# urgent-challenge/urgent2026_challenge_track1

Hardware: AMD Instinct MI355X
Metric: utterances/sec (4 s @ 48 kHz) train step (higher is better)
Workload: dtype bf16

## Files before the change

include/urse.h:

```cpp
#ifndef URSE_H_
#define URSE_H_
#include <stdint.h>

#ifdef __cplusplus
extern "C" {
#endif

#define URSE_OK 0
#define URSE_ERR_INVALID_ARG (-1)
#define URSE_ERR_LAUNCH (-2)
#define URSE_ERR_UNSUPPORTED (-3)
#define URSE_ERR_RUNTIME (-4)

#define URSE_F32 0
#define URSE_BF16 1
#define URSE_F16 2
#define URSE_BF16_ACT_F16 3

#define URSE_WIN_RECT 0
#define URSE_WIN_HANN 1

int urse_version(void);
const char* urse_last_error(void);

#define URSE_KV_NT_BRES 0
#define URSE_KV_NT_RING 1
#define URSE_KV_NT_RING_WIDE 2
#define URSE_KV_NT_128 3
#define URSE_KV_NT_GROUPED_RING 4
#define URSE_KV_NT_GROUPED_128 5
#define URSE_KV_TN_RING 6
#define URSE_KV_TN_RING_T 7
#define URSE_KV_TN_DUAL 8
#define URSE_KV_TN_128 9
#define URSE_KV_TN_GROUPED 10
#define URSE_KV_LSTM_FWD_STREAM 11
#define URSE_KV_LSTM_FWD_WIDE 12
#define URSE_KV_LSTM_FWD_CLUSTER 13
#define URSE_KV_LSTM_FWD_CLUSTER2 14
#define URSE_KV_LSTM_BWD_STREAM16 15
#define URSE_KV_LSTM_BWD_STREAM32 16
#define URSE_KV_LSTM_BWD_CLUSTER 17
#define URSE_KV_LSTM_BWD_SPLIT 18
#define URSE_KV_STFT960 19
#define URSE_KV_STFT_GENERIC 20
#define URSE_KV_ISTFT_GENERIC 21
#define URSE_KV_ISTFT960 22
#define URSE_KV_LSTM_FWD_RW 23
#define URSE_KV_TN_ACT_F16 24
#define URSE_KV_LSTM_FWD_RWX 25
#define URSE_KV_LSTM_BWD_NSPLIT 26
#define URSE_KV_LSTM_FWD_CLUSTERX 27
#define URSE_KV_COUNT 32
int urse_launch_count(int variant);
int urse_launch_counts_reset(void);

int urse_stft_fwd(const float* wav, const int32_t* lens, float* spec, int B, int L, int n_fft, int hop,
                  int window, void* stream);
int urse_istft_fwd(const float* spec, float* wav, int B, int T, int n_fft, int hop, int L_out, int window,
                   void* stream);
int urse_istft_bwd(const float* grad_wav, float* grad_spec, int B, int T, int n_fft, int hop, int L_out,
                   int window, void* stream);

int urse_gemm_nt(const void* A, int64_t lda, const void* B, int64_t ldb, void* C, int64_t ldc, const float* bias,
                 const float* resid, int64_t ldr, int64_t M, int64_t N, int64_t K, int in_dtype, int out_dtype,
                 int act, void* stream);
int urse_gemm_nt_gnstats(const void* A, int64_t lda, const void* B, int64_t ldb, float* C, int64_t ldc, const float* bias,
                         const float* resid, int64_t ldr, int64_t M, int64_t N, int64_t K, int in_dtype, int act,
                         double* stats, int64_t rows_per_group, void* stream);
int urse_gemm_nt_gnbwd(const void* A, int64_t lda, const void* B, int64_t ldb, float* C, int64_t M, int64_t N, int64_t K, int in_dtype,
                       const float* x, const double* stats, const float* gamma, double* sums, float* dgamma, float* dbeta, float* part,
                       int slots, int64_t rows_per_group, float eps, void* stream);
int urse_gemm_nt_grouped(const void* descs, int groups, int max_blocks, int in_dtype, int out_dtype, int act,
                         void* stream);
int urse_gemm_nt_grouped_h(const void* descs, const int64_t* host_descs, int groups, int in_dtype, int out_dtype,
                           int act, void* stream);
int urse_gemm_tn(const void* A, int64_t lda, const void* B, int64_t ldb, float* C, int64_t ldc, float* colsum,
                 int64_t R, int64_t Mo, int64_t No, int64_t shift, int64_t inner, int64_t period,
                 int64_t invalid_step, int64_t perm_h, int dtype, int target_workgroups, void* stream);
int urse_gemm_tn_act_f16_supported(int64_t R, int64_t Mo, int64_t No, int64_t No2, int with_colsum, int64_t inner, int64_t period);
int urse_gemm_tn_dual(const void* A, int64_t lda, const void* B, int64_t ldb, float* C, int64_t ldc, float* colsum,
                      const void* B2, int64_t ldb2, float* C2, int64_t ldc2, int64_t R, int64_t Mo, int64_t No, int64_t No2,
                      int64_t shift, int64_t inner, int64_t period, int64_t invalid_step, int64_t perm_h, int dtype,
                      int target_workgroups, void* stream);
int urse_gemm_tn_grouped(const void* descs, int groups, int max_blocks, int dtype, void* stream);
// ... 196 lines not shown
```

urgent2026_challenge_track1_amd/csrc/gemm.hip:

```cpp
#include <stdlib.h>

#include <type_traits>
#include "urse_common.h"

namespace urse {

typedef __bf16 bf16x8_t __attribute__((ext_vector_type(8)));
typedef short short8_t __attribute__((ext_vector_type(8)));
typedef short short4_t __attribute__((ext_vector_type(4)));
typedef float f32x4_t __attribute__((ext_vector_type(4)));

struct GemmDesc {
  const char* A;
  const char* B;
  char* C;
  const float* bias;
  const float* resid;
  long lda, ldb, ldc;
  long M, N, K;
  long ldr;
};

constexpr int BM = 128, BN = 128;
constexpr int SLAB = 64;
// ... 1150 lines not shown
    ++it_;
#endif
  }
  }
  asm volatile("s_waitcnt vmcnt(0)" ::: "memory");

#pragma unroll
  for (int j = 0; j < NT; ++j) {
    const long v = n0 + (wn * NT + j) * 16 + (lane & 15);
    float* dst = nullptr;
    long ld = 0, col = 0;
    if (v < p.No) { dst = p.C; ld = p.ldc; col = v; }
    else if (v >= No8 && v < V) { dst = p.C2; ld = p.ldc2; col = v - No8; }
    else if (v == vones) { dst = p.colsum; ld = 1; col = 0; }
    if (dst == nullptr) continue;
#pragma unroll
    for (int i = 0; i < MT; ++i)
#pragma unroll
      for (int r = 0; r < 4; ++r) {
        const long row = m0 + wm * (MT * 16) + i * 16 + (lane >> 4) * 4 + r;
        atomicAdd(dst + tn_perm(row, p.perm_h) * ld + col, acc[i][j][r]);
      }
  }
}

static void launch_tn_dma(int ntw, int csm, dim3 grid, hipStream_t st, const TnArgs& p, int cvt = 0) {
  if (cvt == 1) { hipLaunchKernelGGL((gemm_tn_dma_kernel<7, 2, 1>), grid, dim3(512), 0, st, p); return; }
#define URSE_TN_L(N_, C_) hipLaunchKernelGGL((gemm_tn_dma_kernel<N_, C_>), grid, dim3(512), 0, st, p)
  if (ntw == 7) { if (csm == 0) URSE_TN_L(7, 0); else if (csm == 1) URSE_TN_L(7, 1); else URSE_TN_L(7, 2); }
  else { if (csm == 0) URSE_TN_L(8, 0); else if (csm == 1) URSE_TN_L(8, 1); else URSE_TN_L(8, 2); }
#undef URSE_TN_L
}

struct NtExtra {
  double* gstats;
  long rpg;
  const float* gnb_x;
  const double* gnb_stats;
  const float* gnb_gamma;
  double* gnb_sums;
  float* gnb_part;
  int gnb_slots;
  float gnb_eps;
};

template <typename TO, int NTW, int ACT, int BMX, int WNC, int GNB = 0, typename TI = bf16_t>
__device__ __forceinline__ void gemm_nt_dma_body(const GemmDesc& d, double* gstats = nullptr, long rpg = 0, const NtExtra* xt = nullptr) {
  constexpr int BNX = 16 * NTW * WNC, NWV = BMX / 64 * WNC, NTHR = NWV * 64;
  constexpr int BNR = WNC == 2 ? 256 : 16 * NTW * WNC;
  constexpr int NST = NWV == 8 ? URSE_NT_NST : 3, STAGE = (BMX + BNR) * 64, BOFF = BMX * 64;
  constexpr int AI = (BMX / 16 + NWV - 1) / NWV;
  constexpr int BI = (BNR / 16 + NWV - 1) / NWV;
  constexpr int DPW = AI + BI;
  static_assert(AI * NWV * 16 == BMX, "A image blocks divide evenly over the waves");
  __shared__ __attribute__((aligned(1024))) char lds[NST * STAGE + 1024];
  const int tn = (int)((d.N + BNX - 1) / BNX), tm = (int)((d.M + BMX - 1) / BMX);
  if ((int)blockIdx.x >= tm * tn) return;
  const int bid = xcd_remap(blockIdx.x, tm * tn);
  const int tile_m = bid / tn, tile_n = bid - tile_m * tn;
  const long m0 = (long)tile_m * BMX, n0 = (long)tile_n * BNX;
  const int tid = threadIdx.x, lane = tid & 63;
  const int w = __builtin_amdgcn_readfirstlane(tid >> 6), wm = w / WNC, wn = w % WNC;
  const int nk = (int)(d.K / 32);
  const char* zsrc = reinterpret_cast<const char*>(g_tn_zero_page) + lane * 16;
  const int srow = lane >> 2, schunk = (lane & 3) ^ ((lane >> 3) & 3);
  const int lc = lane & 15, lr = lane >> 4;
// ... 175 lines not shown
            uint2 pk;
            pk.x = pack2<TO>(v[0], v[1]);
            pk.y = pack2<TO>(v[2], v[3]);
            *reinterpret_cast<uint2*>(dst) = pk;
          } else {
            *reinterpret_cast<f32x4_t*>(dst) = v;
          }
        }
      }
    }
    __syncthreads();
    if constexpr (GNB) {
      constexpr int SLOTS = NTHR / CPR, XI = (RPP + SLOTS - 1) / SLOTS;
      const int slot = tid / CPR, chf = tid - slot * CPR;
      const long col = n0 + chf * EPC;
#pragma unroll
      for (int i = GXA; i < XI; ++i) {
        const int lr_ = slot + i * SLOTS;
        const long row = m0 + pass * RPP + lr_;
        const bool ok = slot < SLOTS && col < d.N && lr_ < RPP && row < d.M;
        gnb_xpre[i] = ok ? *reinterpret_cast<const float4*>(xt->gnb_x + row * d.ldc + col) : make_float4(0.f, 0.f, 0.f, 0.f);
      }
      if (slot < SLOTS && col < d.N) {
#pragma unroll
        for (int i = 0; i < XI; ++i) {
          const int lr_ = slot + i * SLOTS;
          const long row = m0 + pass * RPP + lr_;
          if (lr_ < RPP && row < d.M) {
            const float4 f = *reinterpret_cast<const float4*>(lds + lr_ * CP + chf * 16);
            __builtin_nontemporal_store(*reinterpret_cast<const f32x4_t*>(&f), reinterpret_cast<f32x4_t*>(C + row * d.ldc + col));
            const float4 xv = gnb_xpre[i];
            const bool first = row < gnb_bound;
            const float mean = first ? gnb_m[0] : gnb_m[1], rstd = first ? gnb_r[0] : gnb_r[1];
            const float dy[4] = {f.x, f.y, f.z, f.w}, xs[4] = {xv.x, xv.y, xv.z, xv.w};
            float a1 = 0.f, a2 = 0.f;
#pragma unroll
            for (int q = 0; q < 4; ++q) {
              const float xh = (xs[q] - mean) * rstd;
              gnb_dg[q] += dy[q] * xh;
              gnb_db[q] += dy[q];
              a1 += dy[q] * gnb_ga[q];
              a2 += dy[q] * gnb_ga[q] * xh;
            }
            if (first) { gsa += a1; gqa += a2; } else { gsb += a1; gqb += a2; }
          }
        }
      }
      continue;
    }
    int lrow = tid / CPR, ch = tid - lrow * CPR;
    constexpr int DROW = NTHR / CPR, DCH = NTHR - DROW * CPR;
    for (; lrow < RPP; lrow += DROW) {
      const long row = m0 + pass * RPP + lrow, col = n0 + ch * EPC;
      if (row < d.M && col < d.N) {
        const char* src = lds + lrow * CP + ch * 16;
        if (vec_ok && col + EPC <= d.N) {
          uint4 v = *reinterpret_cast<const uint4*>(src);
          if (OS == 4 && d.resid && ACT != 2) {
            const float4 rr = *reinterpret_cast<const float4*>(d.resid + row * d.ldr + col);
            float4 f = *reinterpret_cast<float4*>(&v);
            f.x += rr.x; f.y += rr.y; f.z += rr.z; f.w += rr.w;
            v = *reinterpret_cast<uint4*>(&f);
          }
          if (gst) {
            const float4 f = *reinterpret_cast<const float4*>(&v);
            const float sv = (f.x + f.y) + (f.z + f.w), qv = (f.x * f.x + f.y * f.y) + (f.z * f.z + f.w * f.w);
            if (row < gbound) { gsa += sv; gqa += qv; } else { gsb += sv; gqb += qv; }
          }
#ifdef NABL_NO_GST
          if (v.x == 0x12345678u)
#endif
          __builtin_nontemporal_store(*reinterpret_cast<const f32x4_t*>(&v), reinterpret_cast<f32x4_t*>(C + row * d.ldc + col));
          if constexpr (C2K) {
            if (C2) {
              float a0, a1, a2, a3, a4, a5, a6, a7;
              unpack2<f16_t>(v.x, a0, a1); unpack2<f16_t>(v.y, a2, a3); unpack2<f16_t>(v.z, a4, a5); unpack2<f16_t>(v.w, a6, a7);
              const uint4 o = make_uint4(pack2<bf16_t>(a0, a1), pack2<bf16_t>(a2, a3), pack2<bf16_t>(a4, a5), pack2<bf16_t>(a6, a7));
              __builtin_nontemporal_store(*reinterpret_cast<const f32x4_t*>(&o), reinterpret_cast<f32x4_t*>(C2 + row * d.ldr + col));
            }
          }
        } else {
          const TO* sv = reinterpret_cast<const TO*>(src);
          for (int e = 0; e < EPC && col + e < d.N; ++e) {
            float f = to_f32<TO>(sv[e]);
            if (OS == 4 && d.resid && ACT != 2) f += d.resid[row * d.ldr + col + e];
            if (gst) {
              if (row < gbound) { gsa += f; gqa += f * f; } else { gsb += f; gqb += f * f; }
            }
            C[row * d.ldc + col + e] = from_f32<TO>(f);
            if constexpr (C2K) {
              if (C2) C2[row * d.ldr + col + e] = f32_to_bf16(f);
            }
          }
        }
      }
      ch += DCH;
      if (ch >= CPR) { ch -= CPR; ++lrow; }
    }
  }
// ... 30 lines not shown
        const float vg[4] = {sg.x, sg.y, sg.z, sg.w}, vb[4] = {sb.x, sb.y, sb.z, sb.w};
        for (int q = 0; q < 4 && col + q < d.N; ++q) {
          atomicAdd(part + col + q, vg[q]);
          atomicAdd(part + d.N + col + q, vb[q]);
        }
      }
    }
    return;
  }
  if (gst) {
    __syncthreads();
    double* red = reinterpret_cast<double*>(lds);
    const double r0 = wave_sum_d((double)gsa), r1 = wave_sum_d((double)gqa), r2 = wave_sum_d((double)gsb), r3 = wave_sum_d((double)gqb);
    if (lane == 0) { red[w * 4] = r0; red[w * 4 + 1] = r1; red[w * 4 + 2] = r2; red[w * 4 + 3] = r3; }
    __syncthreads();
    if (tid < 4) {
      double t = 0.0;
      for (int i = 0; i < NWV; ++i) t += red[i * 4 + tid];
      const long g = gidx + (tid >> 1);
      if (tid < 2 || gbound < m0 + BMX) {
        if (g * rpg < d.M) atomicAdd(gstats + g * 2 + (tid & 1), t);
      }
    }
  }
}

template <typename TO, int NTW, int ACT, int BMX, int WNC = 2, typename TI = bf16_t>
__global__ void __launch_bounds__(BMX / 64 * WNC * 64) gemm_nt_dma_kernel(GemmDesc d, NtExtra x) {
  gemm_nt_dma_body<TO, NTW, ACT, BMX, WNC, 0, TI>(d, x.gstats, x.rpg);
}

__global__ void __launch_bounds__(512) gemm_nt_dma_gnb_kernel(GemmDesc d, NtExtra x) {
  gemm_nt_dma_body<float, 7, 0, 256, 2, 1>(d, nullptr, 0, &x);
}

__global__ void gnb_fold_kernel(const float* __restrict__ part, int slots, int N, float* __restrict__ dgamma, float* __restrict__ dbeta) {
  const int c = blockIdx.x * blockDim.x + threadIdx.x;
  if (c >= N) return;
  float a = 0.f, b = 0.f;
  for (int s = 0; s < slots; ++s) { a += part[(long)s * 2 * N + c]; b += part[(long)s * 2 * N + N + c]; }
  dgamma[c] += a;
  dbeta[c] += b;
}

template <typename TO, int ACT, typename TI = bf16_t>
__global__ void __launch_bounds__(512) gemm_nt_dma_grouped_kernel(const GemmDesc* __restrict__ descs) {
  const GemmDesc d = descs[blockIdx.y];
  gemm_nt_dma_body<TO, 7, ACT, 256, 2, 0, TI>(d);
}

template <int ACT, typename TI = bf16_t>
__global__ void __launch_bounds__(512) gemm_nt_bres_kernel(GemmDesc d, int wg_per_slice) {
  constexpr int BMX = 256, NTW = 7, BNX = 224, NST = 3, STAGE = BMX * 64, KSTEPS = 7, BRES = KSTEPS * 14 * 1024;
  __shared__ __attribute__((aligned(1024))) char lds[BRES + NST * STAGE];
  char* ring = lds + BRES;
  const int tm = (int)((d.M + BMX - 1) / BMX);
  const int tile_n = blockIdx.x / wg_per_slice, part = blockIdx.x - tile_n * wg_per_slice;
  const long n0 = (long)tile_n * BNX;
  const int tid = threadIdx.x, lane = tid & 63;
  const int w = __builtin_amdgcn_readfirstlane(tid >> 6), wm = w >> 1, wn = w & 1;
  const int nk = (int)(d.K / 32);
  const char* zsrc = reinterpret_cast<const char*>(g_tn_zero_page) + lane * 16;
  const int srow = lane >> 2, schunk = (lane & 3) ^ ((lane >> 3) & 3);
  const int lc = lane & 15, lr = lane >> 4;
  const int foff = lc * 64 + ((lr ^ ((lc >> 1) & 3)) << 4);
  for (int blk = w; blk < nk * 14; blk += 8) {
// ... 253 lines not shown
  URSE_CHECK_ARG(d.A && d.B && d.C, "%s: null operand", who);
  URSE_CHECK_ARG(d.M > 0 && d.N > 0 && d.K > 0, "%s: empty problem", who);
  URSE_CHECK_ARG((d.K * es) % SLAB == 0, "%s: K (%ld) must be a multiple of %d elements", who, d.K, SLAB / es);
  URSE_CHECK_ARG((d.lda * es) % 16 == 0 && (d.ldb * es) % 16 == 0 && ((uintptr_t)d.A % 16) == 0 &&
                     ((uintptr_t)d.B % 16) == 0,
                 "%s: operands must be 16-byte aligned with 16-byte-multiple row pitch", who);
  URSE_CHECK_ARG(d.lda >= d.K && d.ldb >= d.K && d.ldc >= d.N, "%s: leading dimension too small", who);
  return URSE_OK;
}

template <typename T, typename TO>
static void launch_nt(const GemmDesc* descs, const GemmDesc& single, int groups, int max_blocks, int act,
                      hipStream_t st) {
  hipLaunchKernelGGL((gemm_nt_kernel<T, TO>), dim3(max_blocks, 1, groups), dim3(256), 0, st, descs, single, act);
}

static int dispatch_nt(const GemmDesc* descs, const GemmDesc& single, int groups, int max_blocks, int in_dtype,
                       int out_dtype, int act, hipStream_t st) {
  if (in_dtype == URSE_BF16 && out_dtype == URSE_BF16) launch_nt<bf16_t, bf16_t>(descs, single, groups, max_blocks, act, st);
  else if (in_dtype == URSE_BF16 && out_dtype == URSE_F32) launch_nt<bf16_t, float>(descs, single, groups, max_blocks, act, st);
  else if (in_dtype == URSE_F32 && out_dtype == URSE_F32) launch_nt<float, float>(descs, single, groups, max_blocks, act, st);
  else if (in_dtype == URSE_F32 && out_dtype == URSE_BF16) launch_nt<float, bf16_t>(descs, single, groups, max_blocks, act, st);
  else if (in_dtype == URSE_F16 && out_dtype == URSE_F16) launch_nt<f16_t, f16_t>(descs, single, groups, max_blocks, act, st);
  else if (in_dtype == URSE_F16 && out_dtype == URSE_F32) launch_nt<f16_t, float>(descs, single, groups, max_blocks, act, st);
  else { set_error("gemm_nt: bad dtype %d/%d", in_dtype, out_dtype); return URSE_ERR_INVALID_ARG; }
  URSE_CHECK_LAUNCH("urse_gemm_nt");
  return URSE_OK;
}

static long g_nt_bres_min_n = getenv("URSE_NT_BRES_MIN_N") ? atol(getenv("URSE_NT_BRES_MIN_N")) : 448;
static int g_nt_bres_wgs = 256;
static int g_nt_wide_default = 1;
static long g_nt_wide_maxk = 256;

static int gemm_nt_impl(const void* A, int64_t lda, const void* B, int64_t ldb, void* C, int64_t ldc,
                        const float* bias, const float* resid, int64_t ldr, int64_t M, int64_t N, int64_t K,
                        int in_dtype, int out_dtype, int act, void* stream, double* gstats, long rpg, int* fused) {
  NtExtra xtra{};
  GemmDesc d;
  d.A = (const char*)A; d.B = (const char*)B; d.C = (char*)C; d.bias = bias; d.resid = resid;
  d.lda = lda; d.ldb = ldb; d.ldc = ldc; d.M = M; d.N = N; d.K = K; d.ldr = ldr;
  const bool in16 = in_dtype == URSE_BF16 || in_dtype == URSE_F16;
  const bool f16 = in_dtype == URSE_F16;
  URSE_CHECK_ARG(in16 || in_dtype == URSE_F32, "urse_gemm_nt: bad operand dtype %d", in_dtype);
  URSE_CHECK_ARG(out_dtype == URSE_F32 || (out_dtype == URSE_BF16 && !f16) || (out_dtype == URSE_F16 && f16),
                 "urse_gemm_nt: output dtype %d with operand dtype %d (16-bit outputs take the operands' format)", out_dtype, in_dtype);
  const bool out16 = out_dtype != URSE_F32;
  int rc = check_desc_host(d, in16 ? 2 : 4, "urse_gemm_nt");
  if (rc) return rc;
  URSE_CHECK_ARG(!resid || act == 2 || out_dtype == URSE_F32 || (in_dtype == URSE_F16 && out_dtype == URSE_F16 && act == 1),
                 "urse_gemm_nt: residual epilogue writes f32 (f16 operands with act 1: the aux slot is the bf16 copy of the output)");
  URSE_CHECK_ARG(act != 2 || resid, "urse_gemm_nt: act 2 (tanh backward) needs the aux operand");
  static const bool no_dma = getenv("URSE_NT_NO_DMA") != nullptr;
  const char* bres_env = getenv("URSE_NT_BRES");
  const int bres_mode = bres_env ? atoi(bres_env) : 1;
#ifdef URSE_EXPERIMENTS
  const long wreg_min_n = getenv("URSE_NT_WREG_MIN_N") ? atol(getenv("URSE_NT_WREG_MIN_N")) : 0;
  if (wreg_min_n > 0 && in_dtype == URSE_BF16 && out_dtype == URSE_BF16 && !no_dma && M >= 8192 && N >= wreg_min_n && K == 32 * WR_KS &&
      !resid && act != 2 && (ldc * 2) % 16 == 0 && ((uintptr_t)C % 16) == 0 && M * lda * 2 < 0xFFFFF000L && M * ldc * 2 < 0xFFFFF000L) {
    const int tn = (int)((N + WR_BNX - 1) / WR_BNX);
    int parts = 252 / tn;
    if (parts < 1) parts = 1;
    long rpp = (M + parts - 1) / parts;
    rpp = (rpp + WR_ROWS - 1) / WR_ROWS * WR_ROWS;
    dim3 grid((unsigned)(tn * parts));
    hipStream_t st = (hipStream_t)stream;
    note_launch(URSE_KV_NT_BRES);
    if (act == 0) hipLaunchKernelGGL(gemm_nt_wreg_kernel<0>, grid, dim3(448), 0, st, d, parts, rpp);
    else hipLaunchKernelGGL(gemm_nt_wreg_kernel<1>, grid, dim3(448), 0, st, d, parts, rpp);
    URSE_CHECK_LAUNCH("urse_gemm_nt");
    return URSE_OK;
  }
#endif
  if (bres_mode && in16 && out16 && !no_dma && M >= 8192 && N >= g_nt_bres_min_n && K % 32 == 0 &&
      K >= 96 && K <= 224 && !resid && act != 2 && (ldc * 2) % 16 == 0 && ((uintptr_t)C % 16) == 0) {
    const int tn = (int)((N + 223) / 224);
    int per = g_nt_bres_wgs / tn;
    if (per < 1) per = 1;
    dim3 grid((unsigned)(tn * per));
    hipStream_t st = (hipStream_t)stream;
    note_launch(URSE_KV_NT_BRES);
    if (f16) {
      if (act == 0) hipLaunchKernelGGL((gemm_nt_bres_kernel<0, f16_t>), grid, dim3(512), 0, st, d, per);
      else hipLaunchKernelGGL((gemm_nt_bres_kernel<1, f16_t>), grid, dim3(512), 0, st, d, per);
    } else if (act == 0) hipLaunchKernelGGL(gemm_nt_bres_kernel<0>, grid, dim3(512), 0, st, d, per);
    else hipLaunchKernelGGL(gemm_nt_bres_kernel<1>, grid, dim3(512), 0, st, d, per);
    URSE_CHECK_LAUNCH("urse_gemm_nt");
    return URSE_OK;
  }
  if (in16 && !no_dma && M >= 2048 && N >= 160 && K % 32 == 0 && K >= 96 && !(f16 && act == 2)) {
    const long pad7 = (N + 223) / 224 * 224, pad8 = (N + 255) / 256 * 256;
    int ntw = pad7 <= pad8 ? 7 : 8;
    if (const char* e = getenv("URSE_NT_NTW")) ntw = atoi(e) == 8 ? 8 : 7;
    int bmx = 256;
    if (const char* e = getenv("URSE_NT_BMX")) bmx = atoi(e) == 128 ? 128 : 256;
    int wide = g_nt_wide_default && K <= g_nt_wide_maxk && N >= 1792 && out_dtype == URSE_BF16 && (N + 447) / 448 * 448 <= pad7 + 64;
    if (const char* e = getenv("URSE_NT_WIDE")) wide = atoi(e) != 0 && N >= 448;
    if (f16) { wide = 0; bmx = 256; }
    const long tl = wide ? ((M + 127) / 128) * ((N + 447) / 448) : ((M + bmx - 1) / bmx) * ((N + 32L * ntw - 1) / (32L * ntw));
    URSE_CHECK_ARG(tl < (1L << 31), "urse_gemm_nt: too many tiles");
    dim3 grid((unsigned)tl);
    hipStream_t st = (hipStream_t)stream;
    if (gstats && out_dtype == URSE_F32 && act != 2 && !wide && rpg >= bmx) {
      xtra.gstats = gstats;
      xtra.rpg = rpg;
      if (fused) *fused = 1;
    }
#define URSE_NT_DMA(TO_, NTW_, ACT_, BMX_) \
  hipLaunchKernelGGL((gemm_nt_dma_kernel<TO_, NTW_, ACT_, BMX_>), grid, dim3(BMX_ * 2), 0, st, d, xtra)
#define URSE_NT_DMA_W(TO_, ACT_) \
  hipLaunchKernelGGL((gemm_nt_dma_kernel<TO_, 7, ACT_, 128, 4>), grid, dim3(512), 0, st, d, xtra)
#define URSE_NT_DMA_B(TO_, NTW_, ACT_) do { if (wide) URSE_NT_DMA_W(TO_, ACT_); else if (bmx == 128) URSE_NT_DMA(TO_, NTW_, ACT_, 128); else URSE_NT_DMA(TO_, NTW_, ACT_, 256); } while (0)
#define URSE_NT_DMA_ACT(TO_, NTW_) \
  do { if (act == 0) URSE_NT_DMA_B(TO_, NTW_, 0); else if (act == 1) URSE_NT_DMA_B(TO_, NTW_, 1); else URSE_NT_DMA_B(TO_, NTW_, 2); } while (0)
    note_launch(wide ? URSE_KV_NT_RING_WIDE : URSE_KV_NT_RING);
    if (f16) {
#define URSE_NT_DMA_H(TO_, NTW_, ACT_) hipLaunchKernelGGL((gemm_nt_dma_kernel<TO_, NTW_, ACT_, 256, 2, f16_t>), grid, dim3(512), 0, st, d, xtra)
#define URSE_NT_DMA_H_ACT(TO_, NTW_) do { if (act == 0) URSE_NT_DMA_H(TO_, NTW_, 0); else URSE_NT_DMA_H(TO_, NTW_, 1); } while (0)
      if (out_dtype == URSE_F16) { if (ntw == 7) URSE_NT_DMA_H_ACT(f16_t, 7); else URSE_NT_DMA_H_ACT(f16_t, 8); }
      else { if (ntw == 7) URSE_NT_DMA_H_ACT(float, 7); else URSE_NT_DMA_H_ACT(float, 8); }
    } else if (out_dtype == URSE_BF16) {
      if (ntw == 7) URSE_NT_DMA_ACT(bf16_t, 7); else URSE_NT_DMA_ACT(bf16_t, 8);
    } else {
      if (ntw == 7) URSE_NT_DMA_ACT(float, 7); else URSE_NT_DMA_ACT(float, 8);
    }
    URSE_CHECK_LAUNCH("urse_gemm_nt");
    return URSE_OK;
  }
  const long blocks = ((M + BM - 1) / BM) * ((N + BN - 1) / BN);
  URSE_CHECK_ARG(blocks < (1L << 31), "urse_gemm_nt: too many tiles");
  note_launch(URSE_KV_NT_128);
  return dispatch_nt(nullptr, d, 1, (int)blocks, in_dtype, out_dtype, act, (hipStream_t)stream);
}

extern "C" int urse_gemm_nt(const void* A, int64_t lda, const void* B, int64_t ldb, void* C, int64_t ldc,
                            const float* bias, const float* resid, int64_t ldr, int64_t M, int64_t N, int64_t K,
                            int in_dtype, int out_dtype, int act, void* stream) {
  return gemm_nt_impl(A, lda, B, ldb, C, ldc, bias, resid, ldr, M, N, K, in_dtype, out_dtype, act, stream, nullptr, 0, nullptr);
}

extern "C" int urse_gemm_nt_gnstats(const void* A, int64_t lda, const void* B, int64_t ldb, float* C, int64_t ldc,
                                    const float* bias, const float* resid, int64_t ldr, int64_t M, int64_t N, int64_t K,
                                    int in_dtype, int act, double* stats, int64_t rows_per_group, void* stream) {
  URSE_CHECK_ARG(stats && rows_per_group > 0 && M % rows_per_group == 0 && ldc == N && N % 4 == 0,
                 "urse_gemm_nt_gnstats: needs whole groups of rows, a dense output and N %% 4 == 0");
  const int groups = (int)(M / rows_per_group);
  (void)hipMemsetAsync(stats, 0, sizeof(double) * 2 * groups, (hipStream_t)stream);
  int fused = 0;
  int rc = gemm_nt_impl(A, lda, B, ldb, C, ldc, bias, resid, ldr, M, N, K, in_dtype, URSE_F32, act, stream, stats, rows_per_group,
                        &fused);
  if (rc || fused) return rc;
  return urse_groupnorm_stats(C, stats, groups, (int)rows_per_group, 1, (int)N, (int)N, stream);
}

extern "C" int urse_gemm_nt_gnbwd(const void* A, int64_t lda, const void* B, int64_t ldb, float* C, int64_t M, int64_t N, int64_t K,
                                  int in_dtype, const float* x, const double* stats, const float* gamma, double* sums, float* dgamma,
                                  float* dbeta, float* part, int slots, int64_t rows_per_group, float eps, void* stream) {
  URSE_CHECK_ARG(A && B && C && x && stats && gamma && sums && dgamma && dbeta && part && slots > 0 && rows_per_group > 0,
                 "urse_gemm_nt_gnbwd: bad argument");
  static const bool no_dma = getenv("URSE_NT_NO_DMA") != nullptr;
  if (no_dma || in_dtype != URSE_BF16 || M < 2048 || N < 160 || N > 224 || N % 4 || K % 32 || K < 96 || rows_per_group < 256 ||
      M % rows_per_group || ((uintptr_t)C % 16) || ((uintptr_t)x % 16)) {
    set_error("urse_gemm_nt_gnbwd: shape M%ld N%ld K%ld not served by the fused kernel", (long)M, (long)N, (long)K);
    return URSE_ERR_UNSUPPORTED;
  }
  GemmDesc d;
  d.A = (const char*)A; d.B = (const char*)B; d.C = (char*)C; d.bias = nullptr; d.resid = nullptr;
  d.lda = lda; d.ldb = ldb; d.ldc = N; d.M = M; d.N = N; d.K = K; d.ldr = 0;
  int rc = check_desc_host(d, 2, "urse_gemm_nt_gnbwd");
  if (rc) return rc;
  hipStream_t st = (hipStream_t)stream;
  const size_t sums_bytes = sizeof(double) * 2 * (size_t)(M / rows_per_group), part_bytes = sizeof(float) * 2 * (size_t)N * slots;
  if (reinterpret_cast<char*>(part) == reinterpret_cast<char*>(sums) + sums_bytes) {
    (void)hipMemsetAsync(sums, 0, sums_bytes + part_bytes, st);
  } else {
    (void)hipMemsetAsync(sums, 0, sums_bytes, st);
    (void)hipMemsetAsync(part, 0, part_bytes, st);
  }
  NtExtra xt{};
  xt.rpg = rows_per_group; xt.gnb_x = x; xt.gnb_stats = stats; xt.gnb_gamma = gamma; xt.gnb_sums = sums; xt.gnb_part = part;
  xt.gnb_slots = slots; xt.gnb_eps = eps;
  const long tl = (M + 255) / 256;
  URSE_CHECK_ARG(tl < (1L << 31), "urse_gemm_nt_gnbwd: too many tiles");
  note_launch(URSE_KV_NT_RING);
  hipLaunchKernelGGL(gemm_nt_dma_gnb_kernel, dim3((unsigned)tl), dim3(512), 0, st, d, xt);
  hipLaunchKernelGGL(gnb_fold_kernel, dim3((unsigned)((N + 255) / 256)), dim3(256), 0, st, part, slots, (int)N, dgamma, dbeta);
  URSE_CHECK_LAUNCH("urse_gemm_nt_gnbwd");
  return URSE_OK;
}

extern "C" int urse_gemm_nt_grouped(const void* descs, int groups, int max_blocks, int in_dtype, int out_dtype,
                                    int act, void* stream) {
  URSE_CHECK_ARG(descs && groups > 0 && max_blocks > 0, "urse_gemm_nt_grouped: bad argument");
  GemmDesc dummy;
  memset(&dummy, 0, sizeof(dummy));
  note_launch(URSE_KV_NT_GROUPED_128);
  return dispatch_nt((const GemmDesc*)descs, dummy, groups, max_blocks, in_dtype, out_dtype, act,
                     (hipStream_t)stream);
}

extern "C" int urse_gemm_nt_grouped_h(const void* descs, const int64_t* host_descs, int groups, int in_dtype,
                                      int out_dtype, int act, void* stream) {
  URSE_CHECK_ARG(descs && host_descs && groups > 0 && groups < 65536, "urse_gemm_nt_grouped_h: bad argument");
  const GemmDesc* hd = reinterpret_cast<const GemmDesc*>(host_descs);
  const bool f16 = in_dtype == URSE_F16;
  const int es = (in_dtype == URSE_BF16 || f16) ? 2 : 4;
  URSE_CHECK_ARG(out_dtype == URSE_F32 || (out_dtype == URSE_BF16 && !f16) || (out_dtype == URSE_F16 && f16),
                 "urse_gemm_nt_grouped_h: output dtype %d with operand dtype %d", out_dtype, in_dtype);
  bool dma = es == 2 && !(f16 && act == 2) && !getenv("URSE_NT_NO_DMA") && !getenv("URSE_NT_GROUPED_NO_DMA");
  long t128 = 0, tdma = 0;
  const char* mm = getenv("URSE_NT_GROUPED_MIN_M");
  const long min_m = mm ? atol(mm) : 1024;
  for (int g = 0; g < groups; ++g) {
    const GemmDesc& d = hd[g];
    if (int rc = check_desc_host(d, es, "urse_gemm_nt_grouped_h")) return rc;
    dma = dma && d.K % 32 == 0 && d.N >= 160 && d.M >= min_m;
    t128 = std::max(t128, ((d.M + BM - 1) / BM) * ((d.N + BN - 1) / BN));
    tdma = std::max(tdma, ((d.M + 255) / 256) * ((d.N + 223) / 224));
// ... 223 lines not shown
```

urgent2026_challenge_track1_amd/ops.py:

```python
import os

import torch

from . import _lib
from ._lib import call, require_cuda, stream_ptr

WIN_RECT, WIN_HANN = 0, 1
F32, BF16, F16 = 0, 1, 2
BF16_ACT_F16 = 3
HALF_TYPES = (torch.bfloat16, torch.float16)


def bwd_dtype(dtype):
    return torch.bfloat16 if dtype == torch.float16 else dtype

_timing = None


def enable_timing(names):
    global _timing
    _timing = {n: [] for n in names}


def disable_timing():
    global _timing
    t, _timing = _timing, None
    return t


def timed_call(tname, name, *args):
    if _timing is not None and tname in _timing:
        a, b = torch.cuda.Event(enable_timing=True), torch.cuda.Event(enable_timing=True)
        a.record()
        call(name, *args)
        b.record()
        _timing[tname].append((a, b))
    else:
        call(name, *args)


KERNEL_VARIANTS = ("nt_bres", "nt_ring", "nt_ring_wide", "nt_128", "nt_grouped_ring", "nt_grouped_128", "tn_ring", "tn_ring_t",
                   "tn_dual", "tn_128", "tn_grouped", "lstm_fwd_stream", "lstm_fwd_wide", "lstm_fwd_cluster",
                   "lstm_fwd_cluster2", "lstm_bwd_stream16", "lstm_bwd_stream32", "lstm_bwd_cluster", "lstm_bwd_split",
                   "stft960", "stft_generic", "istft_generic", "istft960", "lstm_fwd_rw", "tn_act_f16", "lstm_fwd_rwx", "lstm_bwd_nsplit",
                   "lstm_fwd_clusterx", "_unused28")


_PAGEABLE_UPLOADS = os.environ.get("URSE_PAGEABLE_UPLOADS", "0") == "1"


def upload(host_tensor, device, cached=False):
    if torch.device(device).type != "cuda":
        return host_tensor
    if _PAGEABLE_UPLOADS:
        return host_tensor.to(device)
    out = host_tensor.contiguous().pin_memory().to(device, non_blocking=True)
    if cached:
        ev = torch.cuda.Event()
        ev.record(torch.cuda.current_stream(device))
        ev.synchronize()
    return out


def launch_counts(reset=False):
    lib = _lib.load()
    out = {n: lib.urse_launch_count(i) for i, n in enumerate(KERNEL_VARIANTS)}
    if reset:
        lib.urse_launch_counts_reset()
    return out


def _f32c(t):
    return t.contiguous().float() if (t.dtype != torch.float32 or not t.is_contiguous()) else t


def stft_forward(wav, n_fft, hop, window=WIN_HANN, lens=None):
    require_cuda(wav)
    wav = _f32c(wav)
# ... 154 lines not shown

def groupnorm_fwd(x, gamma, beta, B, T, Kg, W, N, Np, gstride, dtype, eps=1e-5, add=None, stats=None, bf16_copy=False):
    require_cuda(x)
    y = torch.empty(B * T * Kg * (W // N), Np, device=x.device, dtype=dtype)
    y2 = torch.empty_like(y, dtype=torch.bfloat16) if (bf16_copy and dtype == torch.float16) else None
    if stats is not None:
        assert stats.numel() == B * Kg * 2 and stats.dtype == torch.float64
        call("groupnorm_apply", x, gamma, beta, add, y, stats, B, T, Kg, W, N, Np, gstride, float(eps), _dt(y), y2, stream_ptr())
    else:
        stats = torch.empty(B * Kg * 2, device=x.device, dtype=torch.float64)
        call("groupnorm_fwd", x, gamma, beta, add, y, stats, B, T, Kg, W, N, Np, gstride, float(eps), _dt(y), y2, stream_ptr())
    if bf16_copy is None:
        return y, stats, y
    return (y, stats, (y2 if y2 is not None else y)) if bf16_copy else (y, stats)


def groupnorm_bwd(x, dy, stats, gamma, dres, dgamma, dbeta, B, T, Kg, W, N, gstride, eps=1e-5, pack_ld=0, sums=None):
    dx = torch.empty_like(x)
    dxp = torch.empty(x.numel() // N, pack_ld, device=x.device, dtype=torch.bfloat16) if pack_ld else None
    if sums is not None:
        call("groupnorm_bwd_apply", x, dy, stats, sums, gamma, dres, dx, B, T, Kg, W, N, gstride, float(eps), dxp, pack_ld, stream_ptr())
        return (dx, dxp) if pack_ld else dx
    sums = torch.empty(B * Kg * 2, device=x.device, dtype=torch.float64)
    call("groupnorm_bwd", x, dy, stats, gamma, dres, dx, dgamma, dbeta, sums, B, T, Kg, W, N, gstride, float(eps), dxp,
         pack_ld, stream_ptr())
    return (dx, dxp) if pack_ld else dx


FUSE_GN_BWD = os.environ.get("URSE_FUSE_GN_BWD", "1") != "0"
GN_BWD_SLOTS = 16


def gemm_nt_gnbwd_supported(M, N, K, rows_per_group, dtype):
    return (dtype == torch.bfloat16 and M >= 2048 and 160 <= N <= 224 and N % 4 == 0 and K % 32 == 0 and K >= 96 and
            rows_per_group >= 256 and M % rows_per_group == 0 and not os.environ.get("URSE_NT_NO_DMA"))


def gemm_nt_gnbwd(A, W, N, x, stats, gamma, dgamma, dbeta, rows_per_group, eps=1e-5):
    require_cuda(A, W, x)
    M, K = A.shape
    assert W.shape[1] == K and A.stride(1) == 1 and W.stride(1) == 1 and A.dtype == W.dtype and x.is_contiguous() and x.numel() == M * N
    dy = torch.empty(M, N, device=A.device, dtype=torch.float32)
    ng = M // rows_per_group * 2
    ws = torch.empty(ng + GN_BWD_SLOTS * N, device=A.device, dtype=torch.float64)
    sums, part = ws[:ng], ws[ng:].view(torch.float32)
    call("gemm_nt_gnbwd", A, A.stride(0), W, W.stride(0), dy, M, N, K, _dt(A), x, stats, gamma, sums, dgamma, dbeta, part, GN_BWD_SLOTS,
         rows_per_group, float(eps), stream_ptr())
    return dy, sums


LSTM_LAYOUTS = ("whhq", "wihq", "whhb", "wx", "whhTq")
PACK_MULTI_LAYOUTS = {"whhq", "wihq", "whhb", "wx"}


def lstm_layout_ok(name, N, Np, H, Hp, dtype):
    lib = _lib.load()
    if dtype not in HALF_TYPES or Hp % 32:
        return False
    if name == "whhq":
        return True
    if name == "wihq":
        return bool(lib.urse_lstm_clusterx_supported(N, Np, H, Hp))
    if name == "wx":
        return bool(lib.urse_lstm_rwx_supported(N, Np, H, Hp))
    if dtype != torch.bfloat16:
        return False
    if name == "whhb":
# ... 711 lines not shown
```

Baseline: 255.4.

## Add persistent NT ring GEMM kernel with cross-tile prefetch and pipelined epilogue

Adds a persistent variant of the bf16 NT DMA GEMM, used both plain and in the fused GroupNorm-backward form. The grid is capped near the CU count and each workgroup loops over M tiles. The global-to-LDS ring keeps prefetching into the next tile while the current epilogue runs, and the epilogue stages 32-row passes through LDS while prefetching residual or x values a pass ahead. It is on by default except when the plain GEMM has neither a stats nor a residual epilogue. The GN arithmetic is moved into helpers with contraction disabled and explicit fma, and the minimum M for the ring path becomes an environment knob.

Result: no change. 256.5, median of 2 (+0.4%).

```diff
diff --git a/include/urse.h b/include/urse.h
--- a/include/urse.h
+++ b/include/urse.h
@@ -51,6 +51,7 @@
 #define URSE_KV_LSTM_FWD_RWX 25
 #define URSE_KV_LSTM_BWD_NSPLIT 26
 #define URSE_KV_LSTM_FWD_CLUSTERX 27
+#define URSE_KV_NT_RING_PERSIST 28
 #define URSE_KV_COUNT 32
 int urse_launch_count(int variant);
 int urse_launch_counts_reset(void);
diff --git a/urgent2026_challenge_track1_amd/csrc/gemm.hip b/urgent2026_challenge_track1_amd/csrc/gemm.hip
--- a/urgent2026_challenge_track1_amd/csrc/gemm.hip
+++ b/urgent2026_challenge_track1_amd/csrc/gemm.hip
@@ -1206,6 +1206,28 @@
 #undef URSE_TN_L
 }
 
+__device__ __forceinline__ void nt_gst_terms(const float4& f, float& sv, float& qv) {
+#pragma clang fp contract(off)
+  sv = (f.x + f.y) + (f.z + f.w);
+  qv = (f.x * f.x + f.y * f.y) + (f.z * f.z + f.w * f.w);
+}
+__device__ __forceinline__ void nt_gnb_terms(const float4& f, const float4& xv, const float (&ga)[4], float mean, float rstd, float (&dg)[4],
+                                             float (&db)[4], float& a1, float& a2) {
+#pragma clang fp contract(off)
+  const float dy[4] = {f.x, f.y, f.z, f.w}, xs[4] = {xv.x, xv.y, xv.z, xv.w};
+  a1 = 0.f;
+  a2 = 0.f;
+#pragma unroll
+  for (int q = 0; q < 4; ++q) {
+    const float xh = (xs[q] - mean) * rstd;
+    dg[q] = __builtin_fmaf(dy[q], xh, dg[q]);
+    db[q] += dy[q];
+    const float t = dy[q] * ga[q];
+    a1 += t;
+    a2 += t * xh;
+  }
+}
+
 struct NtExtra {
   double* gstats;
   long rpg;
@@ -1447,16 +1469,8 @@
             const float4 xv = gnb_xpre[i];
             const bool first = row < gnb_bound;
             const float mean = first ? gnb_m[0] : gnb_m[1], rstd = first ? gnb_r[0] : gnb_r[1];
-            const float dy[4] = {f.x, f.y, f.z, f.w}, xs[4] = {xv.x, xv.y, xv.z, xv.w};
-            float a1 = 0.f, a2 = 0.f;
-#pragma unroll
-            for (int q = 0; q < 4; ++q) {
-              const float xh = (xs[q] - mean) * rstd;
-              gnb_dg[q] += dy[q] * xh;
-              gnb_db[q] += dy[q];
-              a1 += dy[q] * gnb_ga[q];
-              a2 += dy[q] * gnb_ga[q] * xh;
-            }
+            float a1, a2;
+            nt_gnb_terms(f, xv, gnb_ga, mean, rstd, gnb_dg, gnb_db, a1, a2);
             if (first) { gsa += a1; gqa += a2; } else { gsb += a1; gqb += a2; }
           }
         }
@@ -1479,7 +1493,8 @@
           }
           if (gst) {
             const float4 f = *reinterpret_cast<const float4*>(&v);
-            const float sv = (f.x + f.y) + (f.z + f.w), qv = (f.x * f.x + f.y * f.y) + (f.z * f.z + f.w * f.w);
+            float sv, qv;
+            nt_gst_terms(f, sv, qv);
             if (row < gbound) { gsa += sv; gqa += qv; } else { gsb += sv; gqb += qv; }
           }
 #ifdef NABL_NO_GST
@@ -1576,6 +1591,257 @@
 
 __global__ void __launch_bounds__(512) gemm_nt_dma_gnb_kernel(GemmDesc d, NtExtra x) {
   gemm_nt_dma_body<float, 7, 0, 256, 2, 1>(d, nullptr, 0, &x);
+}
+
+template <int GNB>
+__device__ __forceinline__ void gemm_nt_dma_persist_body(const GemmDesc& d, const NtExtra& xt, int bfull) {
+  constexpr int BMX = 256, NTW = 7, BNX = 224, NWV = 8, NTHR = 512, NST = 4, STAGE = (BMX + 256) * 64, BOFF = BMX * 64;
+  constexpr int PR = 32, NPASS = BMX / PR, CP = BNX * 4 + 16, CPR = BNX / 4;
+  constexpr int SWT = GNB ? (NTHR / CPR) * CPR : NTHR;
+  constexpr int PCH = PR * CPR, XI = (PCH + SWT - 1) / SWT;
+  static_assert(PCH % CPR == 0 && SWT % CPR == 0 || !GNB, "a GNB thread keeps its column chunk");
+  __shared__ __attribute__((aligned(1024))) char lds[NST * STAGE + PR * CP];
+  char* stg = lds + NST * STAGE;
+  const int tiles = (int)((d.M + BMX - 1) / BMX), grid = (int)gridDim.x;
+  const int tid = threadIdx.x, lane = tid & 63;
+  const int w = __builtin_amdgcn_readfirstlane(tid >> 6), wm = w >> 1, wn = w & 1;
+  const int nk = (int)(d.K / 32);
+  const char* zsrc = reinterpret_cast<const char*>(g_tn_zero_page) + lane * 16;
+  const int srow = lane >> 2, schunk = (lane & 3) ^ ((lane >> 3) & 3);
+  const int lc = lane & 15, lr = lane >> 4;
+  const int foff = lc * 64 + ((lr ^ ((lc >> 1) & 3)) << 4);
+  float* C = reinterpret_cast<float*>(d.C);
+
+  const int nbb = bfull ? 16 : (int)((d.N + 15) / 16);
+  const int nbw = __builtin_amdgcn_readfirstlane(nbb - 2 * w >= 2 ? 2 : (nbb - 2 * w == 1 ? 1 : 0));
+  for (int b = nbb + w; b < BNX / 16; b += NWV)
+#pragma unroll
+    for (int s = 0; s < NST; ++s) *reinterpret_cast<uint4*>(lds + s * STAGE + BOFF + b * 1024 + lane * 16) = make_uint4(0u, 0u, 0u, 0u);
+  const char* pb[2];
+  bool bok[2];
+#pragma unroll
+  for (int j = 0; j < 2; ++j) {
+    const int rowl = 16 * (2 * w + j) + srow;
+    bok[j] = rowl < BNX && rowl < d.N;
+    pb[j] = d.B + ((long)rowl * d.ldb) * 2 + schunk * 16;
+  }
+  int it = (int)blockIdx.x, ikt = 0;
+  const char* pa[2];
+  bool aok[2];
+  auto tile_src = [&]() __attribute__((always_inline)) {
+    const long m0i = it < tiles ? (long)xcd_remap(it, tiles) * BMX : 0;
+#pragma unroll
+    for (int j = 0; j < 2; ++j) {
+      const long row = m0i + 16 * (2 * w + j) + srow;
+      aok[j] = it < tiles && row < d.M;
+      pa[j] = d.A + (row * d.lda) * 2 + schunk * 16;
+    }
+  };
+  auto issue_next = [&](int slot) __attribute__((always_inline)) {
+    char* sbase = lds + slot * STAGE;
+#pragma unroll
+    for (int j = 0; j < 2; ++j) glds16(aok[j] ? pa[j] + (long)ikt * 64 : zsrc, sbase + (2 * w + j) * 1024);
+    if (nbw > 0) glds16((it < tiles && bok[0]) ? pb[0] + (long)ikt * 64 : zsrc, sbase + BOFF + (2 * w) * 1024);
+    if (nbw > 1) glds16((it < tiles && bok[1]) ? pb[1] + (long)ikt * 64 : zsrc, sbase + BOFF + (2 * w + 1) * 1024);
+    if (++ikt == nk) { ikt = 0; it += grid; tile_src(); }
+  };
+  tile_src();
+#pragma unroll
+  for (int s = 0; s < NST - 1; ++s) issue_next(s);
+
+  f32x4_t bv[NTW];
+#pragma unroll
+  for (int j = 0; j < NTW; ++j) {
+    const long col = (wn * NTW + j) * 16 + lr * 4;
+#pragma unroll
+    for (int r = 0; r < 4; ++r) bv[j][r] = (!GNB && d.bias && col + r < d.N) ? d.bias[col + r] : 0.f;
+  }
+  const bool gst = !GNB && xt.gstats != nullptr;
+  const bool res = !GNB && d.resid != nullptr;
+  const long rpg = (GNB || gst) ? xt.rpg : 1;
+  float gnb_ga[4] = {0.f, 0.f, 0.f, 0.f};
+  if constexpr (GNB) {
+    const long col = (tid % CPR) * 4;
+#pragma unroll
+    for (int q = 0; q < 4; ++q) gnb_ga[q] = (col + q < d.N) ? xt.gnb_gamma[col + q] : 0.f;
+  }
+  asm volatile("s_waitcnt lgkmcnt(0)" ::: "memory");
+
+  int slot = 0;
+  for (int t = (int)blockIdx.x; t < tiles; t += grid) {
+    const long m0 = (long)xcd_remap(t, tiles) * BMX;
+    f32x4_t acc[4][NTW];
+#pragma unroll
+    for (int i = 0; i < 4; ++i)
+#pragma unroll
+      for (int j = 0; j < NTW; ++j) acc[i][j] = f32x4_t{0.f, 0.f, 0.f, 0.f};
+    for (int kt = 0; kt < nk; ++kt) {
+      if (nbw == 2) asm volatile("s_waitcnt vmcnt(8)" ::: "memory");
+      else if (nbw == 1) asm volatile("s_waitcnt vmcnt(6)" ::: "memory");
+      else asm volatile("s_waitcnt vmcnt(4)" ::: "memory");
+      __builtin_amdgcn_s_barrier();
+      int nslot = slot + NST - 1;
+      if (nslot >= NST) nslot -= NST;
+      issue_next(nslot);
+      const char* As = lds + slot * STAGE + wm * 4096 + foff;
+      const char* Bs = lds + slot * STAGE + BOFF + wn * NTW * 1024 + foff;
+      short8_t a[4];
+#pragma unroll
+      for (int i = 0; i < 4; ++i) a[i] = *reinterpret_cast<const short8_t*>(As + i * 1024);
+      short8_t b[NTW];
+#pragma unroll
+      for (int j = 0; j < NTW; ++j) b[j] = *reinterpret_cast<const short8_t*>(Bs + j * 1024);
+#pragma unroll
+      for (int j = 0; j < NTW; ++j)
+#pragma unroll
+        for (int i = 0; i < 4; ++i) acc[i][j] = Frag<bf16_t>::mma(b[j], a[i], acc[i][j]);
+      if (++slot == NST) slot = 0;
+    }
+
+    float gsa = 0.f, gqa = 0.f, gsb = 0.f, gqb = 0.f;
+    const long gidx = m0 / rpg, gbound = (gidx + 1) * rpg;
+    float gnb_m[2] = {0.f, 0.f}, gnb_r[2] = {0.f, 0.f}, gnb_dg[4] = {0.f, 0.f, 0.f, 0.f}, gnb_db[4] = {0.f, 0.f, 0.f, 0.f};
+    if constexpr (GNB) {
+      const double cnt = (double)rpg * (double)d.N;
+#pragma unroll
+      for (int q = 0; q < 2; ++q) {
+        const long g = (gidx + q) * rpg < d.M ? gidx + q : gidx;
+        const double mu = xt.gnb_stats[g * 2] / cnt;
+        double var = xt.gnb_stats[g * 2 + 1] / cnt - mu * mu;
+        if (var < 0.0) var = 0.0;
+        gnb_m[q] = (float)mu;
+        gnb_r[q] = (float)(1.0 / sqrt(var + (double)xt.gnb_eps));
+      }
+    }
+    const float* esrc = GNB ? xt.gnb_x : d.resid;
+    const long eld = GNB ? d.ldc : d.ldr;
+    const float* ebase = (GNB || res) ? esrc + m0 * eld : nullptr;
+    float* cbase = C + m0 * d.ldc;
+    const int mrem = (int)(d.M - m0 < BMX ? d.M - m0 : BMX), gb = (int)(gbound - m0 < BMX ? gbound - m0 : BMX);
+    const int nn = (int)d.N, ield = (int)eld, ildc = (int)d.ldc;
+    float4 epre[2][XI];
+    auto request = [&](int p, float4 (&dst)[XI]) __attribute__((always_inline)) {
+      int tp = tid;
+      asm volatile("" : "+v"(tp));
+      int r = tp - ((p & 3) * PCH) % SWT;
+      if (r < 0) r += SWT;
+#pragma unroll
+      for (int i = 0; i < XI; ++i) {
+        const int c = r + i * SWT, lrow = c / CPR, ch = c - lrow * CPR, trow = p * PR + lrow;
+        const bool ok = tp < SWT && c < PCH && trow < mrem && ch * 4 < nn;
+        dst[i] = *reinterpret_cast<const float4*>(ebase + (ok ? (unsigned)(trow * ield + ch * 4) : 0u));
+      }
+    };
+    if (GNB || res) request(0, epre[0]);
+#pragma unroll
+    for (int p = 0; p < NPASS; ++p) {
+      if (p + 1 < NPASS && (GNB || res)) request(p + 1, epre[(p + 1) & 1]);
+      if (wm == p / 2) {
+#pragma unroll
+        for (int j = 0; j < NTW; ++j) {
+          const int lcol = (wn * NTW + j) * 16 + lr * 4;
+#pragma unroll
+          for (int ii = 0; ii < 2; ++ii) {
+            const f32x4_t v = acc[2 * (p & 1) + ii][j] + bv[j];
+            *reinterpret_cast<f32x4_t*>(stg + (ii * 16 + lc) * CP + lcol * 4) = v;
+          }
+        }
+      }
+      asm volatile("s_waitcnt lgkmcnt(0)" ::: "memory");
+      __builtin_amdgcn_s_barrier();
+      {
+        int tp = tid;
+        asm volatile("" : "+v"(tp));
+        int r = tp - ((p & 3) * PCH) % SWT;
+        if (r < 0) r += SWT;
+        float4 fs[XI];
+#pragma unroll
+        for (int i = 0; i < XI; ++i) {
+          const int c = r + i * SWT < PCH ? r + i * SWT : PCH - 1, lrow = c / CPR, ch = c - lrow * CPR;
+          fs[i] = *reinterpret_cast<const float4*>(stg + lrow * CP + ch * 16);
+        }
+#pragma unroll
+        for (int i = 0; i < XI; ++i) {
+          const int c = r + i * SWT, lrow = c / CPR, ch = c - lrow * CPR, trow = p * PR + lrow;
+          if (tp < SWT && c < PCH && trow < mrem && ch * 4 < nn) {
+            float4 f = fs[i];
+            const float4 e = epre[p & 1][i];
+            f32x4_t* dst = reinterpret_cast<f32x4_t*>(cbase + (unsigned)(trow * ildc + ch * 4));
+            if constexpr (GNB) {
+              __builtin_nontemporal_store(*reinterpret_cast<const f32x4_t*>(&f), dst);
+              const bool first = trow < gb;
+              const float mean = first ? gnb_m[0] : gnb_m[1], rstd = first ? gnb_r[0] : gnb_r[1];
+              float a1, a2;
+              nt_gnb_terms(f, e, gnb_ga, mean, rstd, gnb_dg, gnb_db, a1, a2);
+              if (first) { gsa += a1; gqa += a2; } else { gsb += a1; gqb += a2; }
+            } else {
+              if (res) { f.x += e.x; f.y += e.y; f.z += e.z; f.w += e.w; }
+              if (gst) {
+                float sv, qv;
+                nt_gst_terms(f, sv, qv);
+                if (trow < gb) { gsa += sv; gqa += qv; } else { gsb += sv; gqb += qv; }
+              }
+              __builtin_nontemporal_store(*reinterpret_cast<const f32x4_t*>(&f), dst);
+            }
+          }
+        }
+      }
+      asm volatile("s_waitcnt lgkmcnt(0)" ::: "memory");
+      __builtin_amdgcn_s_barrier();
+    }
+    if (GNB || gst) {
+      double* red = reinterpret_cast<double*>(stg);
+      float4* pg = reinterpret_cast<float4*>(stg + 1024);
+      float4* pbt = pg + SWT;
+      static_assert(1024 + 2 * SWT * 16 <= PR * CP, "sums fit the staging area");
+      const double r0 = wave_sum_d((double)gsa), r1 = wave_sum_d((double)gqa), r2 = wave_sum_d((double)gsb), r3 = wave_sum_d((double)gqb);
+      if (lane == 0) { red[w * 4] = r0; red[w * 4 + 1] = r1; red[w * 4 + 2] = r2; red[w * 4 + 3] = r3; }
+      if constexpr (GNB) {
+        if (tid < SWT) {
+          pg[tid] = make_float4(gnb_dg[0], gnb_dg[1], gnb_dg[2], gnb_dg[3]);
+          pbt[tid] = make_float4(gnb_db[0], gnb_db[1], gnb_db[2], gnb_db[3]);
+        }
+      }
+      asm volatile("s_waitcnt lgkmcnt(0)" ::: "memory");
+      __builtin_amdgcn_s_barrier();
+      if (tid < 4) {
+        double s = 0.0;
+        for (int i = 0; i < NWV; ++i) s += red[i * 4 + tid];
+        const long g = gidx + (tid >> 1);
+        double* dst = GNB ? xt.gnb_sums : xt.gstats;
+        if ((tid < 2 || gbound < m0 + BMX) && g * rpg < d.M) atomicAdd(dst + g * 2 + (tid & 1), s);
+      }
+      if constexpr (GNB) {
+        if (tid >= 64 && tid < 64 + CPR) {
+          const int chf = tid - 64;
+          const long col = chf * 4;
+          if (col < d.N) {
+            float4 sg = make_float4(0.f, 0.f, 0.f, 0.f), sb = sg;
+            for (int i = 0; i < SWT / CPR; ++i) {
+              const float4 a = pg[i * CPR + chf], bq = pbt[i * CPR + chf];
+              sg.x += a.x; sg.y += a.y; sg.z += a.z; sg.w += a.w;
+              sb.x += bq.x; sb.y += bq.y; sb.z += bq.z; sb.w += bq.w;
+            }
+            float* part = xt.gnb_part + (long)(t % xt.gnb_slots) * 2 * d.N;
+            const float vg[4] = {sg.x, sg.y, sg.z, sg.w}, vb[4] = {sb.x, sb.y, sb.z, sb.w};
+            for (int q = 0; q < 4 && col + q < d.N; ++q) {
+              atomicAdd(part + col + q, vg[q]);
+              atomicAdd(part + d.N + col + q, vb[q]);
+            }
+          }
+        }
+      }
+    }
+  }
+  asm volatile("s_waitcnt vmcnt(0)" ::: "memory");
+}
+
+__global__ void __launch_bounds__(512) gemm_nt_dma_persist_kernel(GemmDesc d, NtExtra x, int bfull) {
+  gemm_nt_dma_persist_body<0>(d, x, bfull);
+}
+
+__global__ void __launch_bounds__(512) gemm_nt_dma_gnb_persist_kernel(GemmDesc d, NtExtra x, int bfull) {
+  gemm_nt_dma_persist_body<1>(d, x, bfull);
 }
 
 __global__ void gnb_fold_kernel(const float* __restrict__ part, int slots, int N, float* __restrict__ dgamma, float* __restrict__ dbeta) {
@@ -1895,6 +2161,25 @@
 static int g_nt_bres_wgs = 256;
 static int g_nt_wide_default = 1;
 static long g_nt_wide_maxk = 256;
+
+static int nt_persist_mode(bool beside_second_queue) {
+  const char* e = getenv("URSE_NT_PERSIST");
+  if (!e) return beside_second_queue ? 0 : 1;
+  const int m = atoi(e);
+  return m == 2 ? 2 : (m != 0);
+}
+static long nt_ring_min_m() {
+  const char* e = getenv("URSE_NT_RING_MIN_M");
+  return e ? atol(e) : 2048;
+}
+static long nt_persist_wgs() {
+  static const long cus = [] {
+    int dev = 0, n = 0;
+    if (hipGetDevice(&dev) != hipSuccess || hipDeviceGetAttribute(&n, hipDeviceAttributeMultiprocessorCount, dev) != hipSuccess || n < 8) n = 256;
+    return (long)(n - n % 8);
+  }();
+  return cus;
+}
 
 static int gemm_nt_impl(const void* A, int64_t lda, const void* B, int64_t ldb, void* C, int64_t ldc,
                         const float* bias, const float* resid, int64_t ldr, int64_t M, int64_t N, int64_t K,
@@ -1951,7 +2236,7 @@
     URSE_CHECK_LAUNCH("urse_gemm_nt");
     return URSE_OK;
   }
-  if (in16 && !no_dma && M >= 2048 && N >= 160 && K % 32 == 0 && K >= 96 && !(f16 && act == 2)) {
+  if (in16 && !no_dma && M >= nt_ring_min_m() && N >= 160 && K % 32 == 0 && K >= 96 && !(f16 && act == 2)) {
     const long pad7 = (N + 223) / 224 * 224, pad8 = (N + 255) / 256 * 256;
     int ntw = pad7 <= pad8 ? 7 : 8;
     if (const char* e = getenv("URSE_NT_NTW")) ntw = atoi(e) == 8 ? 8 : 7;
@@ -1977,6 +2262,16 @@
 #define URSE_NT_DMA_ACT(TO_, NTW_) \
   do { if (act == 0) URSE_NT_DMA_B(TO_, NTW_, 0); else if (act == 1) URSE_NT_DMA_B(TO_, NTW_, 1); else URSE_NT_DMA_B(TO_, NTW_, 2); } while (0)
     note_launch(wide ? URSE_KV_NT_RING_WIDE : URSE_KV_NT_RING);
+    const int persist = nt_persist_mode(!xtra.gstats && !resid);
+    if (persist && in_dtype == URSE_BF16 && out_dtype == URSE_F32 && act == 0 && ntw == 7 && bmx == 256 && !wide && N <= 224 && N % 4 == 0 &&
+        ldc < (1L << 20) && ldr < (1L << 20) && (ldc * 4) % 16 == 0 && ((uintptr_t)C % 16) == 0 &&
+        (!resid || ((ldr * 4) % 16 == 0 && ((uintptr_t)resid % 16) == 0))) {
+      note_launch(URSE_KV_NT_RING_PERSIST);
+      hipLaunchKernelGGL(gemm_nt_dma_persist_kernel, dim3((unsigned)(tl < nt_persist_wgs() ? tl : nt_persist_wgs())), dim3(512), 0, st, d, xtra,
+                         persist == 2);
+      URSE_CHECK_LAUNCH("urse_gemm_nt");
+      return URSE_OK;
+    }
     if (f16) {
 #define URSE_NT_DMA_H(TO_, NTW_, ACT_) hipLaunchKernelGGL((gemm_nt_dma_kernel<TO_, NTW_, ACT_, 256, 2, f16_t>), grid, dim3(512), 0, st, d, xtra)
 #define URSE_NT_DMA_H_ACT(TO_, NTW_) do { if (act == 0) URSE_NT_DMA_H(TO_, NTW_, 0); else URSE_NT_DMA_H(TO_, NTW_, 1); } while (0)
@@ -2022,7 +2317,7 @@
   URSE_CHECK_ARG(A && B && C && x && stats && gamma && sums && dgamma && dbeta && part && slots > 0 && rows_per_group > 0,
                  "urse_gemm_nt_gnbwd: bad argument");
   static const bool no_dma = getenv("URSE_NT_NO_DMA") != nullptr;
-  if (no_dma || in_dtype != URSE_BF16 || M < 2048 || N < 160 || N > 224 || N % 4 || K % 32 || K < 96 || rows_per_group < 256 ||
+  if (no_dma || in_dtype != URSE_BF16 || M < nt_ring_min_m() || N < 160 || N > 224 || N % 4 || K % 32 || K < 96 || rows_per_group < 256 ||
       M % rows_per_group || ((uintptr_t)C % 16) || ((uintptr_t)x % 16)) {
     set_error("urse_gemm_nt_gnbwd: shape M%ld N%ld K%ld not served by the fused kernel", (long)M, (long)N, (long)K);
     return URSE_ERR_UNSUPPORTED;
@@ -2046,7 +2341,13 @@
   const long tl = (M + 255) / 256;
   URSE_CHECK_ARG(tl < (1L << 31), "urse_gemm_nt_gnbwd: too many tiles");
   note_launch(URSE_KV_NT_RING);
-  hipLaunchKernelGGL(gemm_nt_dma_gnb_kernel, dim3((unsigned)tl), dim3(512), 0, st, d, xt);
+  if (const int persist = nt_persist_mode(true)) {
+    note_launch(URSE_KV_NT_RING_PERSIST);
+    hipLaunchKernelGGL(gemm_nt_dma_gnb_persist_kernel, dim3((unsigned)(tl < nt_persist_wgs() ? tl : nt_persist_wgs())), dim3(512), 0, st, d, xt,
+                       persist == 2);
+  } else {
+    hipLaunchKernelGGL(gemm_nt_dma_gnb_kernel, dim3((unsigned)tl), dim3(512), 0, st, d, xt);
+  }
   hipLaunchKernelGGL(gnb_fold_kernel, dim3((unsigned)((N + 255) / 256)), dim3(256), 0, st, part, slots, (int)N, dgamma, dbeta);
   URSE_CHECK_LAUNCH("urse_gemm_nt_gnbwd");
   return URSE_OK;
diff --git a/urgent2026_challenge_track1_amd/ops.py b/urgent2026_challenge_track1_amd/ops.py
--- a/urgent2026_challenge_track1_amd/ops.py
+++ b/urgent2026_challenge_track1_amd/ops.py
@@ -43,7 +43,7 @@
                    "tn_dual", "tn_128", "tn_grouped", "lstm_fwd_stream", "lstm_fwd_wide", "lstm_fwd_cluster",
                    "lstm_fwd_cluster2", "lstm_bwd_stream16", "lstm_bwd_stream32", "lstm_bwd_cluster", "lstm_bwd_split",
                    "stft960", "stft_generic", "istft_generic", "istft960", "lstm_fwd_rw", "tn_act_f16", "lstm_fwd_rwx", "lstm_bwd_nsplit",
-                   "lstm_fwd_clusterx", "_unused28")
+                   "lstm_fwd_clusterx", "nt_ring_persist")
 
 
 _PAGEABLE_UPLOADS = os.environ.get("URSE_PAGEABLE_UPLOADS", "0") == "1"
@@ -264,7 +264,7 @@
 
 
 def gemm_nt_gnbwd_supported(M, N, K, rows_per_group, dtype):
-    return (dtype == torch.bfloat16 and M >= 2048 and 160 <= N <= 224 and N % 4 == 0 and K % 32 == 0 and K >= 96 and
+    return (dtype == torch.bfloat16 and M >= int(os.environ.get("URSE_NT_RING_MIN_M", "2048")) and 160 <= N <= 224 and N % 4 == 0 and K % 32 == 0 and K >= 96 and
             rows_per_group >= 256 and M % rows_per_group == 0 and not os.environ.get("URSE_NT_NO_DMA"))
 
 
```
